# mathematiguy/pypardis

Hardware: AMD Instinct MI355X
Metric: points clustered/sec (whole node), 100M 3-D pts, 1/2/4/8 GPUs; % HBM roofline (higher is better)
Workload: dtype f32 coords, f64 predicate

## Files before the change

pypardis_amd/csrc/engine.hip:

```cpp
#include <cstring>
#include <rocprim/rocprim.hpp>
#ifndef PD_SORT_ROCPRIM
#define PD_SORT_ROCPRIM 0
#endif

#include <algorithm>
#include <type_traits>
#include <cmath>
#include <cstring>
#include <vector>

#include "compact.hpp"
#include "internal.hpp"
#include "pred.hpp"
#include "rsort.hpp"
#include "scan.hpp"
#include "stream.hpp"
#include "uf.hpp"

namespace pd {
namespace {

#ifndef PD_CHECK_BOUNDS
#define PD_CHECK_BOUNDS 0
// ... 525 lines not shown
template <typename K>
__global__ __launch_bounds__(kBlock) void cell_tile_kernel(const K* __restrict__ keys, uint64_t R,
                                                           uint32_t* __restrict__ tile_cnt) {
    uint32_t st[4];
    uint64_t kv[4];
    const uint64_t r0 = ((uint64_t)blockIdx.x * kBlock + threadIdx.x) * 4;
    const uint32_t t = block_sum_u32(cell_starts4<K>(keys, R, r0, st, kv));
    if (threadIdx.x == 0) tile_count_out(tile_cnt, t);
}

template <typename K>
__global__ __launch_bounds__(kBlock) void cell_write_kernel(const K* __restrict__ keys, uint64_t R,
                                                            const uint64_t* __restrict__ tile_off,
                                                            uint32_t* __restrict__ cstart,
                                                            K* __restrict__ ckeys,
                                                            uint32_t* __restrict__ ncells) {
    uint32_t st[4];
    uint64_t kv[4];
    const uint64_t r0 = ((uint64_t)blockIdx.x * kBlock + threadIdx.x) * 4;
    uint32_t btot;
    const uint32_t c = cell_starts4<K>(keys, R, r0, st, kv);
    uint32_t cid = (uint32_t)tile_off[blockIdx.x] + block_excl_scan(c, btot);
#pragma unroll
    for (int q = 0; q < 4; ++q) {
        if (st[q]) {
            cstart[cid] = (uint32_t)(r0 + q);
            ckeys[cid] = (K)kv[q];
        }
        cid += st[q];
        if (r0 + q == R - 1) {
            cstart[cid] = (uint32_t)R;
            *ncells = cid;
        }
    }
}

template <typename WT>
__device__ __forceinline__ WT shfl_up_w(WT x, int o) {
    if constexpr (sizeof(WT) == 4) return (WT)__shfl_up((int)x, o, 64);
    else return (WT)__shfl_up((long long)x, o, 64);
}
template <typename WT>
__device__ __forceinline__ WT shfl_down_w(WT x, int o) {
    if constexpr (sizeof(WT) == 4) return (WT)__shfl_down((int)x, o, 64);
    else return (WT)__shfl_down((long long)x, o, 64);
}
template <typename WT>
__device__ __forceinline__ WT shfl_w(WT x, int l) {
    if constexpr (sizeof(WT) == 4) return (WT)__shfl((int)x, l, 64);
    else return (WT)__shfl((long long)x, l, 64);
}

template <typename K, int SH, bool W32>
__global__ __launch_bounds__(kBlock) void dir_bits_kernel(const K* __restrict__ ckeys,
                                                          const uint32_t* __restrict__ ncells,
                                                          uint4* __restrict__ dir) {
    const uint32_t c = blockIdx.x * kBlock + threadIdx.x;
    const uint32_t nc = *ncells;
    if (c - (uint32_t)(threadIdx.x & 63) >= nc) return;
    const bool in = c < nc;
    using WT = std::conditional_t<W32, uint32_t, uint64_t>;
    const uint64_t k = in ? ((uint64_t)ckeys[c] >> SH) : ~0ull;
    const WT word = (WT)(k >> 6);
    unsigned long long v = in ? (1ull << (k & 63)) : 0ull;
    const int lane = threadIdx.x & 63;
#pragma unroll
    for (int o = 1; o < 64; o <<= 1) {
        const WT wo = shfl_up_w(word, o);
        const unsigned long long vo = (unsigned long long)__shfl_up((long long)v, o, 64);
        if (lane >= o && wo == word) v |= vo;
    }
    const WT wn = shfl_down_w(word, 1);
    const bool last = lane == 63 || wn != word;
    if (in && last) atomicOr(reinterpret_cast<unsigned long long*>(dir + (uint64_t)word), v);
}

template <typename K, bool W32>
__global__ __launch_bounds__(kBlock) void word_write_kernel(const K* __restrict__ ckeys,
                                                            const uint32_t* __restrict__ ncells,
                                                            const uint4* __restrict__ pages,
                                                            uint4* __restrict__ words) {
    const uint32_t c = blockIdx.x * kBlock + threadIdx.x;
    const uint32_t nc = *ncells;
    if (c - (uint32_t)(threadIdx.x & 63) >= nc) return;
    const bool in = c < nc;
    using WT = std::conditional_t<W32, uint32_t, uint64_t>;
    const uint64_t k = in ? (uint64_t)ckeys[c] : ~0ull;
    const WT word = (WT)(k >> 6);
    unsigned long long v = in ? (1ull << (k & 63)) : 0ull;
    const int lane = threadIdx.x & 63;
#pragma unroll
    for (int o = 1; o < 64; o <<= 1) {
        const WT wo = shfl_down_w(word, o);
        const unsigned long long vo = (unsigned long long)__shfl_down((long long)v, o, 64);
        if (lane + o < 64 && wo == word) v |= vo;
    }
    const WT wp = shfl_up_w(word, 1);
    const WT w63 = shfl_w(word, 63);
    const uint32_t cb = c - (uint32_t)lane;
    unsigned long long vx = 0;
    if (cb + 64 < nc && (WT)((uint64_t)ckeys[cb + 64] >> 6) == w63) {
        const uint32_t c2 = cb + 64 + (uint32_t)lane;
        const uint64_t k2 = c2 < nc ? (uint64_t)ckeys[c2] : ~0ull;
        vx = c2 < nc && (WT)(k2 >> 6) == w63 ? 1ull << (k2 & 63) : 0ull;
#pragma unroll
        for (int o = 32; o > 0; o >>= 1) vx |= (unsigned long long)__shfl_xor((long long)vx, o, 64);
    }
    if (!in) return;
    bool first = c == 0;
    if (!first) first = lane ? wp != word : (WT)((uint64_t)ckeys[c - 1] >> 6) != word;
    bool occ;
    const uint64_t slot = page_slot(pages[(uint64_t)word >> 6], (uint64_t)word, occ);
    if (first) {
        if (w63 == word) v |= vx;
        words[slot] = make_uint4((uint32_t)v, (uint32_t)(v >> 32), c, 0u);
    }
    if (c == nc - 1) words[slot + 1] = make_uint4(0u, 0u, nc, 0u);
}

__device__ __forceinline__ uint32_t dir_popc4(const uint4* __restrict__ dir, uint64_t W,
                                              uint64_t w0, uint32_t (&pc)[4]) {
    uint32_t t = 0;
#pragma unroll
    for (int q = 0; q < 4; ++q) {
        pc[q] = 0;
        if (w0 + q < W) {
            const uint4 d = dir[w0 + q];
            pc[q] = (uint32_t)__popc(d.x) + (uint32_t)__popc(d.y);
        }
        t += pc[q];
    }
    return t;
}

__global__ __launch_bounds__(kBlock) void dir_tile_kernel(const uint4* __restrict__ dir, uint64_t W,
                                                          uint32_t* __restrict__ tile_cnt) {
    uint32_t pc[4];
    const uint32_t t =
        block_sum_u32(dir_popc4(dir, W, ((uint64_t)blockIdx.x * kBlock + threadIdx.x) * 4, pc));
    if (threadIdx.x == 0) tile_count_out(tile_cnt, t);
}

__global__ __launch_bounds__(kBlock) void dir_write_kernel(uint4* __restrict__ dir, uint64_t W,
                                                           const uint64_t* __restrict__ tile_off) {
    uint32_t pc[4], btot;
    const uint64_t w0 = ((uint64_t)blockIdx.x * kBlock + threadIdx.x) * 4;
    uint32_t z = (uint32_t)tile_off[blockIdx.x] + block_excl_scan(dir_popc4(dir, W, w0, pc), btot);
#pragma unroll
    for (int q = 0; q < 4; ++q) {
        if (w0 + q < W) dir[w0 + q].z = z;
        z += pc[q];
    }
}

#ifndef PD_INIT_SUB
#define PD_INIT_SUB 16
#endif
constexpr int kInitSub = PD_INIT_SUB;
constexpr uint32_t kInitTile = (uint32_t)kInitSub * kBlock;
static_assert(kInitSub >= 1 && kInitTile * 4 <= 65536, "a block's static LDS");
#ifndef PD_ROOTS_SUB
#define PD_ROOTS_SUB 4
#endif
constexpr int kRootSub = PD_ROOTS_SUB;
constexpr int kRootLists = 64, kRootCntStride = 32;
__global__ __launch_bounds__(kBlock) void init_kernel(uint32_t R, const uint8_t* __restrict__ core,
                                                      const uint32_t* __restrict__ mn,
                                                      int use_mn, uint32_t* __restrict__ par,
                                                      uint32_t* __restrict__ gmin,
                                                      uint32_t* __restrict__ wroot, uint64_t W,
                                                      uint32_t* __restrict__ kbits, uint64_t NW) {
    __shared__ uint32_t lp[kInitTile];
    const uint64_t base = (uint64_t)blockIdx.x * kInitTile;
    uint32_t p[kInitSub];
#pragma unroll
    for (int q = 0; q < kInitSub; ++q) {
        const uint32_t e = (uint32_t)q * kBlock + threadIdx.x;
        const uint64_t r64 = base + e;
        if (r64 < W) wroot[r64] = kNone;
        if (r64 < NW) kbits[r64] = 0u;
        p[q] = kNone;
        if (r64 < R) {
            const uint32_t r = (uint32_t)r64;
            gmin[r] = kNone;
            if (core[r] & 1) {
                p[q] = r;
                if (use_mn) {
                    const uint2 m = reinterpret_cast<const uint2*>(mn)[r];
                    if (m.x < r && (core[m.x] & 1))
                        p[q] = m.x;
                    else if (m.y < r && (core[m.y] & 1))
                        p[q] = m.y;
                }
            }
        }
        lp[e] = p[q];
    }
    if (base >= R) return;
    const uint32_t b32 = (uint32_t)base;
    uint32_t open = 0;
#pragma unroll
    for (int q = 0; q < kInitSub; ++q) {
        const uint32_t e = (uint32_t)q * kBlock + threadIdx.x;
        if (p[q] != kNone && p[q] != b32 + e && p[q] >= b32) open |= 1u << q;
    }
    __syncthreads();
    while (true) {
        uint32_t g[kInitSub];
#pragma unroll
        for (int q = 0; q < kInitSub; ++q) {
            g[q] = p[q];
            if ((open >> q & 1u) && PD_OK(p[q] - b32 < kInitTile, 9, p[q]))
                g[q] = __hip_atomic_load(lp + (p[q] - b32), __ATOMIC_RELAXED,
                                         __HIP_MEMORY_SCOPE_WORKGROUP);
        }
        int moved = 0;
#pragma unroll
        for (int q = 0; q < kInitSub; ++q) {
            if (!(open >> q & 1u)) continue;
            if (g[q] == p[q] || g[q] == kNone) {
                open &= ~(1u << q);
                continue;
            }
            p[q] = g[q];
            __hip_atomic_store(lp + ((uint32_t)q * kBlock + threadIdx.x), g[q], __ATOMIC_RELAXED,
                               __HIP_MEMORY_SCOPE_WORKGROUP);
            moved = 1;
            if (g[q] < b32) open &= ~(1u << q);
        }
        if (!__syncthreads_or(moved)) break;
    }
#pragma unroll
    for (int q = 0; q < kInitSub; ++q) {
        const uint64_t r64 = base + (uint32_t)q * kBlock + threadIdx.x;
        if (r64 < R) par[r64] = p[q];
    }
}

struct LinkStats {
    uint32_t cand = 0, hit = 0, core = 0, same = 0, find_same = 0, unions = 0;
};

__global__ __launch_bounds__(kBlock) void rep_kernel(const uint32_t* __restrict__ list,
                                                     const uint32_t* __restrict__ count,
                                                     const uint32_t* __restrict__ vals,
                                                     const uint32_t* __restrict__ par,
                                                     uint32_t* __restrict__ rep) {
    const uint32_t nl = *count;
    for (uint32_t i = blockIdx.x * kBlock + threadIdx.x; i < nl; i += gridDim.x * kBlock) {
        const uint32_t r = list[i];
        if (par[r] != kNone) atomicMin(rep + (vals[r] & kIdMask), r);
    }
}

__global__ __launch_bounds__(kBlock) void merge_kernel(const uint32_t* __restrict__ list,
                                                       const uint32_t* __restrict__ count,
                                                       const uint32_t* __restrict__ vals,
                                                       const uint32_t* __restrict__ rep,
                                                       uint32_t* __restrict__ par) {
    const uint32_t nl = *count;
    const int lane = threadIdx.x & 63;
    for (uint32_t b0 = blockIdx.x * kBlock; b0 < nl; b0 += gridDim.x * kBlock) {
        const uint32_t i = b0 + threadIdx.x;
        uint32_t ra = kNone, rb = kNone;
        if (i < nl) {
            const uint32_t r = list[i];
            if (ld_rlx(par + r) != kNone) {
                const uint32_t q = rep[vals[r] & kIdMask];
                if (q != r) {
                    ra = uf_find(par, r);
                    rb = uf_find(par, q);
                    if (ra > rb) {
                        const uint32_t t = ra;
                        ra = rb;
                        rb = t;
                    }
                    if (ra == rb) ra = rb = kNone;
                }
            }
        }
        const uint32_t pa = (uint32_t)__shfl_up((int)ra, 1, 64);
        const uint32_t pb = (uint32_t)__shfl_up((int)rb, 1, 64);
        const bool same = lane > 0 && pa == ra && pb == rb;
        if (ra != kNone && !same) uf_unite(par, ra, rb);
    }
}

__global__ __launch_bounds__(kBlock) void roots_kernel(uint32_t R, const uint32_t* __restrict__ vals,
                                                       const uint32_t* __restrict__ gid,
                                                       uint32_t* __restrict__ par,
                                                       uint32_t* __restrict__ gmin,
                                                       uint32_t* __restrict__ rlist,
                                                       uint32_t* __restrict__ rcnt, uint32_t seg,
                                                       uint32_t* __restrict__ counts, int stats) {
    uint32_t ncore = 0;
    uint32_t rr[kRootSub], x0[kRootSub], root[kRootSub], pt[kRootSub];
    bool core[kRootSub];
#pragma unroll
    for (int q = 0; q < kRootSub; ++q) {
        rr[q] = (blockIdx.x * kRootSub + q) * kBlock + threadIdx.x;
        x0[q] = rr[q] < R ? par[rr[q]] : kNone;
        core[q] = x0[q] != kNone;
    }
#pragma unroll
    for (int q = 0; q < kRootSub; ++q) {
        root[q] = core[q] ? par[x0[q]] : 0u;
// ... 1467 lines not shown
    PD_HIP(hipMemcpyFromSymbol(h, HIP_SYMBOL(g_oob), sizeof(h), 0, hipMemcpyDeviceToHost));
    if (h[0]) {
        const unsigned long long z[2] = {0, 0};
        PD_HIP(hipMemcpyToSymbol(HIP_SYMBOL(g_oob), z, sizeof(z), 0, hipMemcpyHostToDevice));
        throw Error(-1, std::string("bounds check failed in ") + kernel + ": " +
                            std::to_string(h[0]) + " violation(s), first at site " +
                            std::to_string(h[1] >> 48) + " index " +
                            std::to_string(h[1] & 0xFFFFFFFFFFFFull));
    }
#else
    (void)s;
    (void)kernel;
#endif
}

template <typename T, int D, typename K, int M>
void run_a(Ctx& ctx, TrainArgs& a, const std::vector<PartGrid>& hparts, uint64_t Gtot,
           int key_bits, EvTimer& tm) {
    hipStream_t s = a.stream;
    const uint64_t n = (uint64_t)a.n;
    const int P = a.P;
    if (Gtot >= (1ull << 53)) throw Error(-5, "eps grid of 2^53 cells or more");
    tm.mark();

    PartGrid* parts = ctx.arena.get<PartGrid>("parts", P);
    const T* X = (const T*)a.X;

    KdTree tree;
    if (!a.owner && a.tree_levels > 0) tree = kd_tree_shape(a.tree_levels, a.tree_sizes, a.tree_cur);
    {
        const size_t pb = (sizeof(PartGrid) * P + 15) & ~size_t(15);
        const size_t tb = tree.nl ? kd_tree_bytes(tree) : 0;
        char* h = (char*)pinned(ctx, pb + tb);
        char* dt = tree.nl ? ctx.arena.get<char>("kd_tree", tb) : nullptr;
        if (tree.nl)
            kd_tree_fill(tree, a.tree_sizes, a.tree_cur, a.tree_axis, a.tree_bound, a.tree_new, D, P,
                         h + pb, dt);
        std::memcpy(h, hparts.data(), sizeof(PartGrid) * P);
        PD_HIP(hipMemcpyAsync(parts, h, sizeof(PartGrid) * P, hipMemcpyHostToDevice, s));
        if (tree.nl) PD_HIP(hipMemcpyAsync(dt, h + pb, tb, hipMemcpyHostToDevice, s));
    }

    const unsigned htiles = (unsigned)std::max<uint64_t>(1, (n + 4 * kBlock - 1) / (4 * kBlock));
    uint32_t* ctrs = ctx.arena.get<uint32_t>("train_ctrs", kCtrs);
    uint32_t* sort_hist = PD_SORT_ROCPRIM ? nullptr : ctx.arena.get<uint32_t>("rsort_hist", 8 * rsort::kRadix);
    uint32_t* tcnt = ctx.arena.get<uint32_t>("tile_cnt", (size_t)htiles + 1);
    uint64_t* toff = ctx.arena.get<uint64_t>("tile_off", (size_t)htiles + 1);
    hipLaunchKernelGGL((halo_tile_kernel<T, D>), dim3(htiles), dim3(kBlock), 0, s, X, n, parts, P,
                       tcnt, ctrs, sort_hist);
    const uint64_t R64 = tile_offsets(ctx, tcnt, htiles, toff, s, true);
    if (R64 >= 0xFFFFFFFEull) throw Error(-5, "more than 2^32-2 halo records on one device");
    K* keys = ctx.arena.get<K>("keys", R64);
    uint32_t* vals = ctx.arena.get<uint32_t>("vals", R64);
    if (P <= 64)
        hipLaunchKernelGGL((halo_write_kernel<T, D, K, true>), dim3(htiles), dim3(kBlock), 0, s, X,
                           n, parts, P, a.owner, tree, toff, R64, keys, vals);
    else
        hipLaunchKernelGGL((halo_write_kernel<T, D, K, false>), dim3(htiles), dim3(kBlock), 0, s, X,
                           n, parts, P, a.owner, tree, toff, R64, keys, vals);
    PD_HIP(hipGetLastError());
    check_bounds(s, "halo_write_kernel");
    const uint32_t R = (uint32_t)R64;
    ctx.t.records = R;
    K* keys2 = ctx.arena.get<K>("keys2", R);
    uint32_t* vals2 = ctx.arena.get<uint32_t>("vals2", R);
    tm.mark();

    T* Xs = ctx.arena.get<T>("Xs", (size_t)R * Stride<D>::v);
    uint32_t* dup_list = ctx.arena.get<uint32_t>("dup_list", R);
    uint32_t* lcount = ctrs;
    uint32_t* rep = P > 1 ? ctx.arena.get<uint32_t>("rep", n) : nullptr;
    sort_records<K>(ctx, keys, vals, keys2, vals2, (uint64_t)R, key_bits, s,
                    !PD_SORT_ROCPRIM);
    tm.mark();
    hipLaunchKernelGGL((gather_kernel<T, D>), dim3(blocks(R)), dim3(kBlock), 0, s, X, (uint64_t)R,
                       vals, Xs, dup_list, lcount, rep);
    uint64_t* wrec = nullptr;
    uint32_t* wbad = nullptr;
    if (a.weight) {
        uint64_t* wfix = ctx.arena.get<uint64_t>("weight_fix", n);
        wrec = ctx.arena.get<uint64_t>("weight_rec", R);
        wbad = ctx.arena.get<uint32_t>("weight_bad", 4);
        PD_HIP(hipMemsetAsync(wbad, 0, sizeof(uint32_t), s));
        hipLaunchKernelGGL(weight_fix_kernel, dim3(blocks(n)), dim3(kBlock), 0, s, a.weight, n, wfix,
                           wbad);
        if (R)
            hipLaunchKernelGGL(record_weight_kernel, dim3(blocks(R)), dim3(kBlock), 0, s, wfix, vals,
                               (uint64_t)R, n, wrec);
        PD_HIP(hipGetLastError());
        check_bounds(s, "record_weight_kernel");
    }
    tm.mark();

#ifndef PD_NC_SYNC
#define PD_NC_SYNC 1
#endif
    uint32_t* part_start = ctx.arena.get<uint32_t>("part_start", P + 1);
    hipLaunchKernelGGL((part_start_kernel<K>), dim3((P + 1 + 63) / 64), dim3(64), 0, s, keys,
                       (uint64_t)R, parts, P, part_start);
    uint32_t* cstart = ctx.arena.get<uint32_t>("cstart", (size_t)R + 1);
    K* ckeys = ctx.arena.get<K>("cell_keys", (size_t)R + 1);
    uint32_t* dncells = ctx.arena.get<uint32_t>("ncells", 4);
    if (R) {
        const unsigned ctiles = (unsigned)((R + 4 * kBlock - 1) / (4 * kBlock));
        uint32_t* ccnt = ctx.arena.get<uint32_t>("tile_cnt", (size_t)ctiles + 1);
        uint64_t* coff = ctx.arena.get<uint64_t>("tile_off", (size_t)ctiles + 1);
        hipLaunchKernelGGL((cell_tile_kernel<K>), dim3(ctiles), dim3(kBlock), 0, s, keys,
                           (uint64_t)R, ccnt);
        tile_offsets(ctx, ccnt, ctiles, coff, s, false);
        hipLaunchKernelGGL((cell_write_kernel<K>), dim3(ctiles), dim3(kBlock), 0, s, keys,
                           (uint64_t)R, coff, cstart, ckeys, dncells);
    } else {
        PD_HIP(hipMemsetAsync(cstart, 0, sizeof(uint32_t), s));
        PD_HIP(hipMemsetAsync(dncells, 0, sizeof(uint32_t), s));
    }
    uint64_t cgrid0 = R;
#if PD_NC_SYNC
    if (R) {
        uint32_t* hnc = (uint32_t*)((char*)pinned(ctx, 16) + 8);
        PD_HIP(hipMemcpyAsync(hnc, dncells, sizeof(uint32_t), hipMemcpyDeviceToHost, s));
        uint32_t* hwb = hnc + 1;
        if (wbad) PD_HIP(hipMemcpyAsync(hwb, wbad, sizeof(uint32_t), hipMemcpyDeviceToHost, s));
        sync(s);
        cgrid0 = std::max<uint64_t>(1, std::min<uint64_t>(*hnc, R));
        if (wbad && *hwb)
            throw Error(-1, "sample_weight: " + std::to_string(*hwb) +
                                " value(s) not finite or outside [0, 2^31]");
        wbad = nullptr;
    }
#endif
    if (wbad) {
        uint32_t* hwb = (uint32_t*)pinned(ctx, sizeof(uint32_t));
        PD_HIP(hipMemcpyAsync(hwb, wbad, sizeof(uint32_t), hipMemcpyDeviceToHost, s));
        sync(s);
        if (*hwb)
            throw Error(-1, "sample_weight: " + std::to_string(*hwb) +
                                " value(s) not finite or outside [0, 2^31]");
    }
    auto prefix_words = [&](uint4* d, uint64_t nw, bool read_total) -> uint64_t {
        const unsigned wtiles = (unsigned)std::max<uint64_t>(1, (nw + 4 * kBlock - 1) / (4 * kBlock));
        uint32_t* wcnt = ctx.arena.get<uint32_t>("tile_cnt", (size_t)wtiles + 1);
        uint64_t* woff = ctx.arena.get<uint64_t>("tile_off", (size_t)wtiles + 1);
        hipLaunchKernelGGL(dir_tile_kernel, dim3(wtiles), dim3(kBlock), 0, s, d, nw, wcnt);
        const uint64_t tot = tile_offsets(ctx, wcnt, wtiles, woff, s, read_total);
        hipLaunchKernelGGL(dir_write_kernel, dim3(wtiles), dim3(kBlock), 0, s, d, nw, woff);
        return tot;
    };
    uint64_t W;
    uint4* dir;
    uint4* pages = nullptr;
    if (!a.dir_paged) {
        W = (Gtot >> 6) + 2;
        dir = ctx.arena.get<uint4>("dir", W);
        PD_HIP(hipMemsetAsync(dir, 0, sizeof(uint4) * W, s));
        if (R) {
            if (sizeof(K) == 4 || key_bits <= 37)
                hipLaunchKernelGGL((dir_bits_kernel<K, 0, true>), dim3(blocks(cgrid0)), dim3(kBlock), 0, s,
                                   ckeys, dncells, dir);
            else
                hipLaunchKernelGGL((dir_bits_kernel<K, 0, false>), dim3(blocks(cgrid0)), dim3(kBlock), 0,
                                   s, ckeys, dncells, dir);
        }
        prefix_words(dir, W, false);
    } else {
        const uint64_t NP = (Gtot >> 12) + 2;
        pages = ctx.arena.get<uint4>("dir_pages", NP);
        PD_HIP(hipMemsetAsync(pages, 0, sizeof(uint4) * NP, s));
        if (R) {
            if (sizeof(K) == 4 || key_bits <= 43)
                hipLaunchKernelGGL((dir_bits_kernel<K, 6, true>), dim3(blocks(cgrid0)), dim3(kBlock), 0, s,
                                   ckeys, dncells, pages);
            else
                hipLaunchKernelGGL((dir_bits_kernel<K, 6, false>), dim3(blocks(cgrid0)), dim3(kBlock), 0,
                                   s, ckeys, dncells, pages);
        }
        if (R && !PD_NC_SYNC)
            PD_HIP(hipMemcpyAsync((char*)pinned(ctx, 16) + 8, dncells, sizeof(uint32_t),
                                  hipMemcpyDeviceToHost, s));
        const uint64_t nw = prefix_words(pages, NP, true);
        W = nw + 1;
        dir = ctx.arena.get<uint4>("dir", W);
        if (R)
        {
            const uint32_t nch = *(const uint32_t*)((const char*)pinned(ctx, 16) + 8);
            const uint64_t wg = std::max<uint64_t>(1, std::min<uint64_t>(nch, R));
            if (sizeof(K) == 4 || key_bits <= 37)
                hipLaunchKernelGGL((word_write_kernel<K, true>), dim3(blocks(wg)), dim3(kBlock), 0, s,
                                   ckeys, dncells, pages, dir);
            else
                hipLaunchKernelGGL((word_write_kernel<K, false>), dim3(blocks(wg)), dim3(kBlock), 0, s,
                                   ckeys, dncells, pages, dir);
        }
        else
            PD_HIP(hipMemsetAsync(dir, 0, sizeof(uint4), s));
    }
    ctx.t.dir_words = (int64_t)W;
    PD_HIP(hipGetLastError());
    tm.mark();

    Cells C{parts, part_start, P, dir, cstart, pages};
    const double eps = a.eps, eps2 = a.eps * a.eps;
    float slo = -1.0f, shi = INFINITY;
    {
        const double thr = a.metric == 0 ? eps2 : eps;
        if (std::is_same<T, float>::value && thr > 1e-30 && thr < 1e30 && ctx.screen) {
            slo = std::nextafter((float)(thr * (1.0 - 1.0 / 262144.0)), 0.0f);
            shi = std::nextafter((float)(thr * (1.0 + 1.0 / 262144.0)), INFINITY);
        }
    }
    uint8_t* core = ctx.arena.get<uint8_t>("core", R);
    uint32_t* mn = ctx.arena.get<uint32_t>("minnbr", 2 * (size_t)R);
    uint32_t* cnt_rec = a.counts ? ctx.arena.get<uint32_t>("cnt_rec", R) : nullptr;
    unsigned long long* sst = nullptr;
    if (ctx.sweep_stats) {
        sst = ctx.arena.get<unsigned long long>("sweep_stats", 10);
        PD_HIP(hipMemsetAsync(sst, 0, sizeof(unsigned long long) * 10, s));
    }
    uint32_t* h_nc = nullptr;
    hipEvent_t ev_nc = nullptr;
    if (R && ctx.centre_window < 0) {
        h_nc = (uint32_t*)pinned(ctx, sizeof(uint32_t));
        PD_HIP(hipEventCreateWithFlags(&ev_nc, hipEventDisableTiming));
        PD_HIP(hipMemcpyAsync(h_nc, dncells, sizeof(uint32_t), hipMemcpyDeviceToHost, s));
        PD_HIP(hipEventRecord(ev_nc, s));
    }
    if (R) {
        const uint32_t rot = ctx.count_rotate ? (uint32_t)ctx.count_rotate : 0xFFFFFFFFu;
        if (wrec)
            launch_count_weighted<T, D, M>(s, Xs, R, C, eps, eps2, slo, shi, (uint32_t)a.min_samples,
                                           ctx.full_counts ? 1 : 0, rot, core, mn, wrec);
        else if (sst)
            launch_count<T, D, M, true>(s, Xs, R, C, eps, eps2, slo, shi, (uint32_t)a.min_samples,
                                        ctx.full_counts ? 1 : 0, rot, core, mn, cnt_rec, sst);
        else
            launch_count<T, D, M, false>(s, Xs, R, C, eps, eps2, slo, shi, (uint32_t)a.min_samples,
                                         ctx.full_counts ? 1 : 0, rot, core, mn, cnt_rec, sst);
        if (ctx.count_replay > 0 && !sst && !wrec)
            ctx.t.count_kernel = replay_count<T, D, M>(
                s, Xs, R, (uint32_t)ctx.count_replay, C, eps, eps2, slo, shi,
                (uint32_t)a.min_samples, ctx.full_counts ? 1 : 0, rot, core, mn, cnt_rec);
    }
    PD_HIP(hipGetLastError());
    tm.mark();

    uint32_t* par = ctx.arena.get<uint32_t>("parent", R);
    uint32_t* gmin = ctx.arena.get<uint32_t>("gmin", R);
    if (R) {
        uint32_t* wroot = ctx.arena.get<uint32_t>("word_root", W);
        const uint64_t NW = a.phase == 0 ? (n + 31) / 32 : 0;
        const uint64_t NWz = NW ? ((NW + 31) & ~uint64_t(31)) + kRootLists * kRootCntStride : 0;
        uint32_t* kbits = NW ? ctx.arena.get<uint32_t>("key_bits", NWz) : nullptr;
        hipLaunchKernelGGL(init_kernel,
                           dim3(sub_blocks(std::max<uint64_t>(std::max<uint64_t>(R, W), NWz), kInitSub)),
                           dim3(kBlock), 0, s, R, core, mn, 1, par, gmin, wroot, (uint64_t)W, kbits, NWz);
        check_bounds(s, "init_kernel");
        int cw = ctx.centre_window;
        uint64_t cgrid = R;
        if (cw < 0) {
            PD_HIP(hipEventSynchronize(ev_nc));
            (void)hipEventDestroy(ev_nc);
            const uint32_t nc = *h_nc ? *h_nc : 1u;
            cgrid = std::min<uint64_t>(nc, R);
            cw = 2 * (uint64_t)R <= 5ull * nc ? 2 : ((uint64_t)R <= 8ull * nc ? 8 : 16);
        }
        auto go = [&](auto Wc) {
            constexpr int Wv = decltype(Wc)::value;
            constexpr int Kw = window_groups((int)sizeof(T), D, Wv);
            const unsigned wb = blocks(((uint64_t)R + Kw - 1) / Kw);
            if (sst)
                hipLaunchKernelGGL((window_uf_kernel<T, D, M, Wv, true>), dim3(wb), dim3(kBlock), 0,
                                   s, Xs, R, eps, eps2, slo, shi, par, sst);
            else
                hipLaunchKernelGGL((window_uf_kernel<T, D, M, Wv, false>), dim3(wb), dim3(kBlock), 0,
                                   s, Xs, R, eps, eps2, slo, shi, par, sst);
        };
        if (cw <= 2)
            go(std::integral_constant<int, 2>{});
        else if (cw <= 4)
            go(std::integral_constant<int, 4>{});
        else if (cw <= 8)
            go(std::integral_constant<int, 8>{});
        else if (cw <= 16)
            go(std::integral_constant<int, 16>{});
        else if (cw <= 32)
            go(std::integral_constant<int, 32>{});
        else
            go(std::integral_constant<int, 64>{});
        uint32_t* croot = ctx.arena.get<uint32_t>("cell_root", R);
        {
            uint32_t* big = ctx.arena.get<uint32_t>("big_cells", R / (kWordBig + 1) + 1);
            uint32_t* mid = ctx.arena.get<uint32_t>("mid_cells", R / (kMidCell + 1) + 1);
            uint32_t* nbig = ctrs + 8;
            if ((uint64_t)W < 0xFFFFFFFFull)
                hipLaunchKernelGGL((cell_word_root_kernel<K, true>), dim3(blocks(cgrid)), dim3(kBlock), 0,
                                   s, cstart, dncells, ckeys, par, croot, wroot, mid, nbig + 1, big,
                                   nbig, pages);
            else
                hipLaunchKernelGGL((cell_word_root_kernel<K, false>), dim3(blocks(cgrid)), dim3(kBlock),
                                   0, s, cstart, dncells, ckeys, par, croot, wroot, mid, nbig + 1,
                                   big, nbig, pages);
            hipLaunchKernelGGL((mid_cell_word_root_kernel<K>), dim3(2048), dim3(kBlock), 0, s,
                               cstart, ckeys, mid, nbig + 1, par, croot, wroot, pages);
            hipLaunchKernelGGL((big_cell_word_root_kernel<K>), dim3(1024), dim3(kBlock), 0, s,
                               cstart, ckeys, big, nbig, par, croot, wroot, pages);
        }
        const uint32_t pcap = (uint32_t)std::min<uint64_t>(R, 64ull << 20);
        uint2* plist = ctx.arena.get<uint2>("pair_list", pcap);
        uint32_t* pcount = ctrs + 10;
        const unsigned vtiles = blocks(cgrid);
        uint8_t* vflag = ctx.arena.get<uint8_t>("verify_flags", R);
        uint32_t* vlist = ctx.arena.get<uint32_t>("verify_list", R);
        uint32_t* vcnt = ctx.arena.get<uint32_t>("tile_cnt", (size_t)vtiles + 1);
        uint64_t* voff = ctx.arena.get<uint64_t>("tile_off", (size_t)vtiles + 1);
        if (ctx.verify_fused) {
            hipLaunchKernelGGL((cell_verify_kernel<T, D, M, K>), dim3(vtiles), dim3(kBlock), 0, s,
                               Xs, keys, nullptr, 0u, croot, wroot, C, xsub_of(ctx), eps, eps2,
// ... 544 lines not shown
```

Measured before the change: 4.425 billion.

## Build flat cell directory in one pass from sorted keys, skipping memset and scan

Replaces the memset + bit-scatter + two-kernel prefix scan for the non-paged directory with a single kernel that derives each directory word's occupancy bits and starting cell index directly from the sorted cell keys via wave shuffles and binary search. Long empty stretches are queued to a gap list and filled by a separate grid-strided kernel, so each word is written once instead of being zeroed, scattered, reread and rewritten. This adds a gap-capacity counter and atomic appends, and a compile-time check mode compares against the old path.

```diff
diff --git a/pypardis_amd/csrc/engine.hip b/pypardis_amd/csrc/engine.hip
--- a/pypardis_amd/csrc/engine.hip
+++ b/pypardis_amd/csrc/engine.hip
@@ -701,6 +701,135 @@
         z += pc[q];
     }
 }
+
+#ifndef PD_DIR_GAP
+#define PD_DIR_GAP 1024
+#endif
+constexpr uint32_t kDirGap = PD_DIR_GAP;
+static_assert(kDirGap >= 64 && (kDirGap & (kDirGap - 1)) == 0,
+              "a power of two; the sweep's jump needs a long gap to outrun one 64-word step");
+constexpr int kDirGapCtr = 11;
+constexpr uint32_t kDirGapChunk = 4096;
+constexpr unsigned kDirGapBlocks = 1024;
+
+__device__ __forceinline__ void dir_gap_append(uint64_t* __restrict__ gaps,
+                                               uint32_t* __restrict__ gap_cnt, uint32_t gap_cap,
+                                               uint64_t w0, uint64_t nw, uint32_t z) {
+    const uint32_t g = atomicAdd(gap_cnt, 1u);
+    if (PD_OK(g < gap_cap, 10, g) && g < gap_cap) {
+        gaps[3 * (uint64_t)g] = w0;
+        gaps[3 * (uint64_t)g + 1] = nw;
+        gaps[3 * (uint64_t)g + 2] = z;
+    }
+}
+
+template <typename K, bool W32>
+__global__ __launch_bounds__(kBlock) void dir_flat_kernel(const K* __restrict__ ckeys,
+                                                          const uint32_t* __restrict__ ncells,
+                                                          uint4* __restrict__ dir, uint64_t W,
+                                                          uint64_t* __restrict__ gaps,
+                                                          uint32_t* __restrict__ gap_cnt,
+                                                          uint32_t gap_cap) {
+    const uint32_t c = blockIdx.x * kBlock + threadIdx.x;
+    const uint32_t nc = *ncells;
+    const int lane = threadIdx.x & 63;
+    const uint32_t cb = c - (uint32_t)lane;
+    if (cb >= nc) return;
+    const bool in = c < nc;
+    using WT = std::conditional_t<W32, uint32_t, uint64_t>;
+    const uint64_t k = in ? (uint64_t)ckeys[c] : ~0ull;
+    const WT word = (WT)(k >> 6);
+    unsigned long long v = in ? (1ull << (k & 63)) : 0ull;
+#pragma unroll
+    for (int o = 1; o < 64; o <<= 1) {
+        const WT wo = shfl_down_w(word, o);
+        const unsigned long long vo = (unsigned long long)__shfl_down((long long)v, o, 64);
+        if (lane + o < 64 && wo == word) v |= vo;
+    }
+    const WT wp = shfl_up_w(word, 1);
+    const WT w63 = shfl_w(word, 63);
+    if (cb + 64 < nc && (WT)((uint64_t)ckeys[cb + 64] >> 6) == w63) {
+        const uint32_t c2 = cb + 64 + (uint32_t)lane;
+        const uint64_t k2 = c2 < nc ? (uint64_t)ckeys[c2] : ~0ull;
+        unsigned long long vx = c2 < nc && (WT)(k2 >> 6) == w63 ? 1ull << (k2 & 63) : 0ull;
+#pragma unroll
+        for (int o = 32; o > 0; o >>= 1) vx |= (unsigned long long)__shfl_xor((long long)vx, o, 64);
+        if (word == w63) v |= vx;
+    }
+    const uint32_t nv = nc - cb < 64u ? nc - cb : 64u;
+    const WT hi = shfl_w(word, (int)nv - 1);
+    const WT lo = cb ? (WT)((uint64_t)ckeys[cb - 1] >> 6) + 1 : (WT)0;
+    const WT lo_j = lane ? wp + 1 : lo;
+    const bool first = in && word >= lo_j;
+    const bool lng = first && word - lo_j > (WT)kDirGap;
+    if (lng) dir_gap_append(gaps, gap_cnt, gap_cap, (uint64_t)lo_j, (uint64_t)(word - lo_j), c);
+    const unsigned long long lmask = __ballot(lng);
+    for (WT base = lo; base <= hi;) {
+        const WT w = base + (WT)lane;
+        int j = 0;
+#pragma unroll
+        for (int st = 32; st > 0; st >>= 1)
+            if (shfl_w(word, j + st - 1) < w) j += st;
+        const WT wj = shfl_w(word, j);
+        const unsigned long long vj = (unsigned long long)__shfl((long long)v, j, 64);
+        const bool occ = wj == w;
+        const bool skip = w <= hi && !occ && (lmask >> j & 1ull);
+        if (w <= hi && !skip && PD_OK((uint64_t)w < W, 11, w) && (uint64_t)w < W)
+            dir[(uint64_t)w] = make_uint4(occ ? (uint32_t)vj : 0u, occ ? (uint32_t)(vj >> 32) : 0u,
+                                          cb + (uint32_t)j, 0u);
+        if (__ballot(skip) >> 63) base = shfl_w(wj, 63);
+        else base += 64;
+    }
+    if (cb + 64 >= nc) {
+        const uint64_t t0 = (uint64_t)hi + 1;
+        const uint64_t tn = W > t0 ? W - t0 : 0;
+        if (tn > kDirGap) {
+            if (lane == 0) dir_gap_append(gaps, gap_cnt, gap_cap, t0, tn, nc);
+        } else {
+            for (uint64_t i = (uint64_t)lane; i < tn; i += 64) dir[t0 + i] = make_uint4(0u, 0u, nc, 0u);
+        }
+    }
+}
+
+__global__ __launch_bounds__(kBlock) void dir_gap_kernel(const uint64_t* __restrict__ gaps,
+                                                         const uint32_t* __restrict__ gap_cnt,
+                                                         uint32_t gap_cap, uint4* __restrict__ dir,
+                                                         uint64_t W) {
+    const uint32_t cnt = *gap_cnt;
+    const uint32_t ng = cnt < gap_cap ? cnt : gap_cap;
+    for (uint32_t g = 0; g < ng; ++g) {
+        const uint64_t w0 = gaps[3 * (uint64_t)g];
+        uint64_t nw = gaps[3 * (uint64_t)g + 1];
+        const uint32_t z = (uint32_t)gaps[3 * (uint64_t)g + 2];
+        (void)PD_OK(w0 <= W && nw <= W - w0, 12, w0);
+        nw = w0 >= W ? 0 : nw < W - w0 ? nw : W - w0;
+        const uint64_t nch = (nw + kDirGapChunk - 1) / kDirGapChunk;
+        for (uint64_t ch = (blockIdx.x + gridDim.x - g % gridDim.x) % gridDim.x; ch < nch;
+             ch += gridDim.x) {
+            const uint64_t e = nw < (ch + 1) * kDirGapChunk ? nw : (ch + 1) * kDirGapChunk;
+            for (uint64_t i = ch * kDirGapChunk + threadIdx.x; i < e; i += kBlock)
+                dir[w0 + i] = make_uint4(0u, 0u, z, 0u);
+        }
+    }
+}
+
+#ifndef PD_DIR_SCAN
+#define PD_DIR_SCAN 0
+#endif
+#ifndef PD_DIR_CHECK
+#define PD_DIR_CHECK 0
+#endif
+#if PD_DIR_CHECK
+__global__ __launch_bounds__(kBlock) void dir_cmp_kernel(const uint4* __restrict__ got,
+                                                         const uint4* __restrict__ want, uint64_t W,
+                                                         unsigned long long* __restrict__ bad) {
+    for (uint64_t w = (uint64_t)blockIdx.x * kBlock + threadIdx.x; w < W;
+         w += (uint64_t)gridDim.x * kBlock) {
+        const uint4 a = got[w], b = want[w];
+        if (a.x != b.x || a.y != b.y || a.z != b.z || a.w != b.w) atomicMin(bad, (unsigned long long)w);
+    }
+}
+#endif
 
 #ifndef PD_INIT_SUB
 #define PD_INIT_SUB 16
@@ -2474,16 +2603,66 @@
     if (!a.dir_paged) {
         W = (Gtot >> 6) + 2;
         dir = ctx.arena.get<uint4>("dir", W);
-        PD_HIP(hipMemsetAsync(dir, 0, sizeof(uint4) * W, s));
-        if (R) {
-            if (sizeof(K) == 4 || key_bits <= 37)
-                hipLaunchKernelGGL((dir_bits_kernel<K, 0, true>), dim3(blocks(cgrid0)), dim3(kBlock), 0, s,
-                                   ckeys, dncells, dir);
+        const bool w32 = sizeof(K) == 4 || key_bits <= 37;
+#if PD_DIR_SCAN || PD_DIR_CHECK
+        auto flat_scan = [&](uint4* d) {
+            PD_HIP(hipMemsetAsync(d, 0, sizeof(uint4) * W, s));
+            if (R) {
+                if (w32)
+                    hipLaunchKernelGGL((dir_bits_kernel<K, 0, true>), dim3(blocks(cgrid0)),
+                                       dim3(kBlock), 0, s, ckeys, dncells, d);
+                else
+                    hipLaunchKernelGGL((dir_bits_kernel<K, 0, false>), dim3(blocks(cgrid0)),
+                                       dim3(kBlock), 0, s, ckeys, dncells, d);
+            }
+            prefix_words(d, W, false);
+        };
+#endif
+#if PD_DIR_SCAN
+        flat_scan(dir);
+#else
+        if (!R) {
+            PD_HIP(hipMemsetAsync(dir, 0, sizeof(uint4) * W, s));
+        } else {
+            const uint32_t gap_cap =
+                (uint32_t)std::min<uint64_t>(W / kDirGap + (uint64_t)P + 2, (uint64_t)R + 2);
+            uint64_t* gaps = ctx.arena.get<uint64_t>("dir_gaps", 3 * (size_t)gap_cap);
+            uint32_t* gap_cnt = ctrs + kDirGapCtr;
+            if (w32)
+                hipLaunchKernelGGL((dir_flat_kernel<K, true>), dim3(blocks(cgrid0)), dim3(kBlock), 0, s,
+                                   ckeys, dncells, dir, W, gaps, gap_cnt, gap_cap);
             else
-                hipLaunchKernelGGL((dir_bits_kernel<K, 0, false>), dim3(blocks(cgrid0)), dim3(kBlock), 0,
-                                   s, ckeys, dncells, dir);
-        }
-        prefix_words(dir, W, false);
+                hipLaunchKernelGGL((dir_flat_kernel<K, false>), dim3(blocks(cgrid0)), dim3(kBlock), 0, s,
+                                   ckeys, dncells, dir, W, gaps, gap_cnt, gap_cap);
+            hipLaunchKernelGGL(dir_gap_kernel, dim3(kDirGapBlocks), dim3(kBlock), 0, s, gaps, gap_cnt,
+                               gap_cap, dir, W);
+            PD_HIP(hipGetLastError());
+            check_bounds(s, "dir_flat_kernel");
+#if PD_DIR_CHECK
+            uint4* want = ctx.arena.get<uint4>("dir_check", W);
+            unsigned long long* bad = ctx.arena.get<unsigned long long>("dir_check_bad", 1);
+            flat_scan(want);
+            PD_HIP(hipMemsetAsync(bad, 0xFF, sizeof(unsigned long long), s));
+            hipLaunchKernelGGL(dir_cmp_kernel, dim3(2048), dim3(kBlock), 0, s, dir, want, W, bad);
+            PD_HIP(hipGetLastError());
+            unsigned long long hb = 0;
+            PD_HIP(hipMemcpyAsync(&hb, bad, sizeof(hb), hipMemcpyDeviceToHost, s));
+            sync(s);
+            if (hb != ~0ull) {
+                uint4 g, w;
+                PD_HIP(hipMemcpyAsync(&g, dir + hb, sizeof(g), hipMemcpyDeviceToHost, s));
+                PD_HIP(hipMemcpyAsync(&w, want + hb, sizeof(w), hipMemcpyDeviceToHost, s));
+                sync(s);
+                auto str = [](const uint4& q) {
+                    return "{" + std::to_string(q.x) + ", " + std::to_string(q.y) + ", " +
+                           std::to_string(q.z) + ", " + std::to_string(q.w) + "}";
+                };
+                throw Error(-1, "directory check failed: word " + std::to_string(hb) + " of " +
+                                    std::to_string(W) + ": got " + str(g) + ", want " + str(w));
+            }
+#endif
+        }
+#endif
     } else {
         const uint64_t NP = (Gtot >> 12) + 2;
         pages = ctx.arena.get<uint4>("dir_pages", NP);
```

New measurement: 4.512 billion (median of 6 runs). +2.0%, better.
